# tjiiv-cprg/EPro-PnP

Hardware: AMD Instinct MI355X
Metric: PnP instances/sec (fwd+bwd, N=512 pts, 512 samples) (higher is better)
Workload: dtype f32; 1 GPU; C2 batched synthetic: 4096 objects/GPU x N=512 points, S=512 MC samples, K=4 AMIS iters, L=3 LM iters, EProPnP6DoF fwd+bwd; objects_per_gpu=4096, objects_total=4096, num_points=512, mc_samples=512, amis_iters=4, lm_iters=3, dof=6, parallelism=objects sharded x1, no data-path collective

## Files before the change

### epro-pnp_amd/csrc/amis_backward_mfma.hip

```cpp
#include "amis_common.h"
#include "dispatch.h"
#include "tuning.h"

namespace pnp {

template <int DOF, bool BOUNDS, int NPT, bool BF16>
constexpr int bwd_min_waves() { return (NPT <= 2) ? PNP_BWD_MINW : PNP_BWD_MINW4; }

template <int DOF, bool BOUNDS, int NPT, bool BF16 = false>
__global__ __launch_bounds__(512, (bwd_min_waves<DOF, BOUNDS, NPT, BF16>())) void amis_backward_mfma_kernel(Problem p, const float* __restrict__ pose_samples,
                                                                     const float* __restrict__ g_logw, int S,
                                                                     const float* __restrict__ pose_init,
                                                                     const float* __restrict__ g_init, int P16,
                                                                     float* __restrict__ gx3d, float* __restrict__ gx2d,
                                                                     float* __restrict__ gw2d, float* __restrict__ gdelta,
                                                                     int nsplit, float drop_eps, int gw_rows) {
  constexpr int PL = PoseLen<DOF>::value;
  typedef ProjOp<BF16> Proj;
  const int v = object_of_block(p.B * nsplit);
  if (v >= p.B * nsplit) return;
  const int b = v / nsplit, part = v - b * nsplit;
  const int T = (int)blockDim.x, tid = (int)threadIdx.x, lane = lane_id(), wv = wave_id(), W = T >> 6;

  PNP_PHASES_BEGIN(6);
  PNP_DYN_SMEM(float, smem);
  float* ptab = smem;
  float* wtab = ptab + 12 * P16;
  float* wraw = wtab + P16;
  int* idx = reinterpret_cast<int*>(wraw + P16);
  float* red = reinterpret_cast<float*>(idx + P16);
  float* hist = red + 80;
  float* gwl = hist + kDropHistFloats;
  const bool fold = (p.delta_stats != nullptr) && (nsplit == 1);
  const bool park = fold && (gw_rows >= p.N);

  float Kc[9], delta;
  Bounds bd;
  load_camera<BOUNDS>(p, b, Kc, bd, delta);
  const HuberScale hs = huber_scale(delta);
  const float zmin_v = to_vgpr(p.z_min), one_v = to_vgpr(1.0f);
  const float front_scale = to_vgpr(0x1p60f);
  const float front_off = to_vgpr(-nextafterf(p.z_min, -1.0f) * 0x1p60f);
  const float tiny_v = to_vgpr(1e-30f);

  const bool with_init = (pose_init != nullptr) && (g_init != nullptr);
  const int P = S + (with_init ? 1 : 0);
  const float g_init_b = with_init ? g_init[b] : 0.f;

  float amax = 0.f;
  for (int m = tid; m < P; m += T) {
    const float w = (m < S) ? -g_logw[(size_t)m * p.B + b] : g_init_b;
    wraw[m] = w;
    if (m < S) amax = fmaxf(amax, fabsf(w));
  }
  amax = block_max(amax, red);
  __syncthreads();
  PNP_PHASE(0);
  const float askip = mass_drop_threshold([&](int m) { return fabsf(wraw[m]); }, S, amax, drop_eps, hist);
  for (int m = tid; m < S; m += T)
    if (fabsf(wraw[m]) <= askip) wraw[m] = 0.f;
  __syncthreads();
  PNP_PHASE(1);
  if (wv == 0) {
    const int seg = (P + 63) >> 6;
    const int m0 = lane * seg, m1 = min(P, m0 + seg);
    int cnt = 0;
    for (int m = m0; m < m1; ++m) cnt += (wraw[m] != 0.f) ? 1 : 0;
    int* lcnt = reinterpret_cast<int*>(red);
    lcnt[lane] = cnt;
    wave_lds_fence();
    int off = 0, total = 0;
    for (int l = 0; l < 64; ++l) {
      const int c = lcnt[l];
      off += (l < lane) ? c : 0;
      total += c;
    }
    for (int m = m0; m < m1; ++m)
      if (wraw[m] != 0.f) idx[off++] = m;
    if (lane == 0) lcnt[64] = total;
  }
  __syncthreads();
  PNP_PHASE(2);
  const int nact = reinterpret_cast<const int*>(red)[64];
  const int ntile = (nact + 15) >> 4;
  for (int c = tid; c < ntile * 16; c += T) {
    float* dst = ptab + (c >> 2) * 48 + (c & 3);
    if (c < nact) {
      const int m = idx[c];
      const float* src = (m < S) ? pose_samples + ((size_t)m * p.B + b) * PL : pose_init + (size_t)b * PL;
      float ps[PL], R[9], KR[9], Kt[3];
#pragma unroll
      for (int i = 0; i < PL; ++i) ps[i] = src[i];
      pose_to_rot<DOF>(ps, R);
      compose_kr_kt(Kc, R, ps, KR, Kt);
#pragma unroll
      for (int r = 0; r < 3; ++r) {
        dst[(4 * r + 0) * 4] = KR[3 * r]; dst[(4 * r + 1) * 4] = KR[3 * r + 1]; dst[(4 * r + 2) * 4] = KR[3 * r + 2];
        dst[(4 * r + 3) * 4] = Kt[r];
      }
      wtab[c] = wraw[m];
    } else {
#pragma unroll
      for (int k = 0; k < 12; ++k) dst[k * 4] = (k == 11) ? 1.f : 0.f;
      wtab[c] = 0.f;
    }
  }
  __syncthreads();
  PNP_PHASE(3);

  const int col = lane & 15, kk = lane >> 4, g4 = kk * 4;
  float gd = 0.f;
  const int chunk_pts = W * NPT * 16;
  for (int c0 = part * chunk_pts; c0 < p.N; c0 += nsplit * chunk_pts) {
    typename Proj::T rB[NPT];
    float4 rW[NPT];
    f32x2 A1x[NPT], A1y[NPT], A2x[NPT], A2y[NPT];
    f32x2 gXv[NPT], gYv[NPT], gZv[NPT];
#pragma unroll
    for (int i = 0; i < NPT; ++i) {
      const Point q = load_point(p, b, c0 + (wv + W * i) * 16 + col);
      rB[i] = Proj::b((kk == 0) ? q.X : (kk == 1) ? q.Y : (kk == 2) ? q.Z : 1.0f);
      const float wu = q.wu * hs.inv_delta, wv = q.wv * hs.inv_delta;
      rW[i] = make_float4(wu, -q.u * wu, wv, -q.v * wv);
      A1x[i] = A1y[i] = A2x[i] = A2y[i] = f32x2{0.f, 0.f};
      gXv[i] = gYv[i] = gZv[i] = f32x2{0.f, 0.f};
    }
    f32x2 gsat2 = {0.f, 0.f};
    const floatx4 zero = {0.f, 0.f, 0.f, 0.f};
    const f32x2 tiny2 = {tiny_v, tiny_v};
    for (int t = 0; t < ntile; ++t) {
      const float* grp = ptab + (t * 4 + (col >> 2)) * 48 + (col & 3);
      const typename Proj::T ax = Proj::a(grp[kk * 4]), ay = Proj::a(grp[(4 + kk) * 4]), az = Proj::a(grp[(8 + kk) * 4]);
      const float4 aw4 = *reinterpret_cast<const float4*>(wtab + t * 16 + g4);
      const float4* rows = reinterpret_cast<const float4*>(ptab + (t * 4 + kk) * 48);
      const float4 kxx = rows[0], kxy = rows[1], kxz = rows[2], kyx = rows[4], kyy = rows[5], kyz = rows[6], kzx = rows[8], kzy = rows[9],
                   kzz = rows[10];
      constexpr bool kPipe = (NPT == 4);
      floatx4 hxn = zero, hyn = zero, hzn = zero;
      if (kPipe) {
        hxn = Proj::mma(ax, rB[0], zero); hyn = Proj::mma(ay, rB[0], zero); hzn = Proj::mma(az, rB[0], zero);
      }
#pragma unroll
      for (int i = 0; i < NPT; ++i) {
        floatx4 hx, hy, hz;
        if (kPipe) {
          hx = hxn; hy = hyn; hz = hzn;
          if (i + 1 < NPT) {
            hxn = Proj::mma(ax, rB[i + 1], zero);
            hyn = Proj::mma(ay, rB[i + 1], zero);
            hzn = Proj::mma(az, rB[i + 1], zero);
            sched_fence();
          }
        } else {
          hx = Proj::mma(ax, rB[i], zero);
          hy = Proj::mma(ay, rB[i], zero);
          hz = Proj::mma(az, rB[i], zero);
        }
        const float4 w4 = rW[i];
        const f32x2 wu2 = {w4.x, w4.x}, cu2 = {w4.y, w4.y}, wv2 = {w4.z, w4.z}, cv2 = {w4.w, w4.w};
#pragma unroll
        for (int h = 0; h < 2; ++h) {
          const f32x2 hx2 = {hx[2 * h], hx[2 * h + 1]}, hy2 = {hy[2 * h], hy[2 * h + 1]};
          const float hz0 = hz[2 * h], hz1 = hz[2 * h + 1];
          const f32x2 aw2 = h ? f32x2{aw4.z, aw4.w} : f32x2{aw4.x, aw4.y};
          const f32x2 rz2 = {fast_rcp(clamp_below(hz0, zmin_v)), fast_rcp(clamp_below(hz1, zmin_v))};
          f32x2 rx2, ry2, ghx2, ghy2, ghz2;
          f32x2 coef2, crx2, cry2;
          if (!BOUNDS) {
            const f32x2 wrx2 = rz2 * wu2, wry2 = rz2 * wv2;
            rx2 = fma2(hx2, wrx2, cu2);
            ry2 = fma2(hy2, wry2, cv2);
            const f32x2 s22 = fma2(rx2, rx2, fma2(ry2, ry2, tiny2));
            const f32x2 c12 = {sat_mul(fast_rsqrt(s22[0]), one_v), sat_mul(fast_rsqrt(s22[1]), one_v)};
            coef2 = aw2 * c12;
            gsat2 = fma2(aw2, f32x2{sat_mul(s22[0], one_v), sat_mul(s22[1], one_v)}, gsat2);
            crx2 = coef2 * rx2;
            cry2 = coef2 * ry2;
            ghx2 = crx2 * wrx2;
            ghy2 = cry2 * wry2;
            ghz2 = -rz2 * fma2(ghx2, hx2, ghy2 * hy2);
          } else {
            const f32x2 ppx2 = hx2 * rz2, ppy2 = hy2 * rz2;
            const f32x2 px2 = {clamp_lu(ppx2[0], bd.lbx, bd.ubx), clamp_lu(ppx2[1], bd.lbx, bd.ubx)};
            const f32x2 py2 = {clamp_lu(ppy2[0], bd.lby, bd.uby), clamp_lu(ppy2[1], bd.lby, bd.uby)};
            rx2 = fma2(px2, wu2, cu2);
            ry2 = fma2(py2, wv2, cv2);
            const f32x2 s22 = fma2(rx2, rx2, fma2(ry2, ry2, tiny2));
            const f32x2 c12 = {sat_mul(fast_rsqrt(s22[0]), one_v), sat_mul(fast_rsqrt(s22[1]), one_v)};
            coef2 = aw2 * c12;
            gsat2 = fma2(aw2, f32x2{sat_mul(s22[0], one_v), sat_mul(s22[1], one_v)}, gsat2);
            crx2 = coef2 * rx2;
            cry2 = coef2 * ry2;
            f32x2 gpx2 = crx2 * wu2, gpy2 = cry2 * wv2;
            gpx2 = f32x2{(px2[0] == ppx2[0]) ? gpx2[0] : 0.f, (px2[1] == ppx2[1]) ? gpx2[1] : 0.f};
            gpy2 = f32x2{(py2[0] == ppy2[0]) ? gpy2[0] : 0.f, (py2[1] == ppy2[1]) ? gpy2[1] : 0.f};
            ghx2 = gpx2 * rz2;
            ghy2 = gpy2 * rz2;
            ghz2 = fma2(-ghx2, ppx2, -(ghy2 * ppy2));
          }
          ghz2 = ghz2 * f32x2{sat_fma(hz0, front_scale, front_off), sat_fma(hz1, front_scale, front_off)};
          A2x[i] = fma2(crx2, rx2, A2x[i]);
          A2y[i] = fma2(cry2, ry2, A2y[i]);
          A1x[i] = fma2(coef2, rx2, A1x[i]);
          A1y[i] = fma2(coef2, ry2, A1y[i]);
          const f32x2 kxx2 = h ? f32x2{kxx.z, kxx.w} : f32x2{kxx.x, kxx.y}, kyx2 = h ? f32x2{kyx.z, kyx.w} : f32x2{kyx.x, kyx.y},
                      kzx2 = h ? f32x2{kzx.z, kzx.w} : f32x2{kzx.x, kzx.y};
          const f32x2 kxy2 = h ? f32x2{kxy.z, kxy.w} : f32x2{kxy.x, kxy.y}, kyy2 = h ? f32x2{kyy.z, kyy.w} : f32x2{kyy.x, kyy.y},
                      kzy2 = h ? f32x2{kzy.z, kzy.w} : f32x2{kzy.x, kzy.y};
          const f32x2 kxz2 = h ? f32x2{kxz.z, kxz.w} : f32x2{kxz.x, kxz.y}, kyz2 = h ? f32x2{kyz.z, kyz.w} : f32x2{kyz.x, kyz.y},
                      kzz2 = h ? f32x2{kzz.z, kzz.w} : f32x2{kzz.x, kzz.y};
          gXv[i] = fma2(kxx2, ghx2, fma2(kyx2, ghy2, fma2(kzx2, ghz2, gXv[i])));
          gYv[i] = fma2(kxy2, ghx2, fma2(kyy2, ghy2, fma2(kzy2, ghz2, gYv[i])));
          gZv[i] = fma2(kxz2, ghx2, fma2(kyz2, ghy2, fma2(kzz2, ghz2, gZv[i])));
        }
      }
    }
    const float gsat = gsat2[0] + gsat2[1];
    {
      float a2 = 0.f;
#pragma unroll
      for (int i = 0; i < NPT; ++i) a2 += (A2x[i][0] + A2x[i][1]) + (A2y[i][0] + A2y[i][1]);
      gd += a2 - gsat;
    }
    const int laneE = (int)f32_bits(to_vgpr(bits_f32((unsigned)lane)));
    const int colE = laneE & 15, g4E = (laneE >> 4) * 4;
    const float ind0 = (colE == 0) ? 1.f : 0.f, ind1 = (colE == 1) ? 1.f : 0.f, ind2 = (colE == 2) ? 1.f : 0.f,
                ind3 = (colE == 3) ? 1.f : 0.f;
#pragma unroll
    for (int i = 0; i < NPT; ++i) {
      floatx4 D1 = zero;
      D1 = mfma_16x16x4((gXv[i][0] + gXv[i][1]) * hs.delta_sq, ind0, D1);
      D1 = mfma_16x16x4((gYv[i][0] + gYv[i][1]) * hs.delta_sq, ind1, D1);
      D1 = mfma_16x16x4((gZv[i][0] + gZv[i][1]) * hs.delta_sq, ind2, D1);
      const float4 w4 = rW[i];
      floatx4 D2 = zero;
      const float a1x = A1x[i][0] + A1x[i][1], a1y = A1y[i][0] + A1y[i][1], a2x = A2x[i][0] + A2x[i][1], a2y = A2y[i][0] + A2y[i][1];
      D2 = mfma_16x16x4(-w4.x * a1x * hs.delta_sq, ind0, D2);
      D2 = mfma_16x16x4(-w4.z * a1y * hs.delta_sq, ind1, D2);
      D2 = mfma_16x16x4((w4.x != 0.f) ? a2x * hs.delta / w4.x : 0.f, ind2, D2);
      D2 = mfma_16x16x4((w4.z != 0.f) ? a2y * hs.delta / w4.z : 0.f, ind3, D2);
      const int nb = c0 + (wv + W * i) * 16 + g4E;
#pragma unroll
      for (int r = 0; r < 4; ++r) {
        const int n = nb + r;
        if (n < p.N) {
          const size_t o = (size_t)b * p.N + n;
          if (colE < 3) gx3d[o * 3 + colE] = D1[r];
          if (colE < 2) gx2d[o * 2 + colE] = D2[r];
          else if (colE < 4) {
            if (park) gwl[n * 2 + (colE - 2)] = D2[r]; else gw2d[o * 2 + (colE - 2)] = D2[r];
          }
        }
      }
    }
  }
  PNP_PHASE(4);
  float one[1] = {gd * hs.delta};
  block_sum<1>(one, red);
  if (tid == 0) gdelta[v] = one[0];
  if (fold) {
    const float add = (one[0] * p.delta_stats[(size_t)b * 4 + 1]) * (p.delta_relative / (2.0f * (float)p.N));
    __syncthreads();
    float* row = gw2d + (size_t)b * p.N * 2;
    if (park) {
      for (int i = tid; i < 2 * p.N; i += T) row[i] = gwl[i] + add;
    } else {
      for (int i = tid; i < 2 * p.N; i += T) row[i] += add;
    }
  }
  PNP_PHASE(5);
  PNP_PHASES_FLUSH(6);
}

int tuning_bwd_phase_cycles(unsigned long long* out, int reset) { return tuning::read_cycles(out, reset, false); }

template <class F>
static int dispatch_bwd_npt(int npt, F&& f) {
  switch (npt) {
    case 1: return f(ic<1>{});
    case 2: return f(ic<2>{});
    default: return f(ic<4>{});
  }
}

struct BwdPlan {
  int waves, npt, P16, gw_rows;
  size_t smem;
  bool bf16;
};

static int plan_amis_backward(const epropnp_problem* prob, int mc_samples, bool with_init, int nsplit, BwdPlan* out) {
  const int B = prob->num_obj, N = prob->num_pts;
  const int P = mc_samples + (with_init ? 1 : 0);
  const int P16 = ((P + 15) / 16) * 16 + 16;
  size_t smem = sizeof(float) * (15 * (size_t)P16 + 80 + kDropHistFloats);
  if (smem > 160 * 1024) return 1;
  int gw_rows = 0;
  if (prob->delta_stats != nullptr && nsplit == 1 && 3 * (smem + sizeof(float) * 2 * (size_t)N) <= 160 * 1024) {
    gw_rows = N;
    smem += sizeof(float) * 2 * (size_t)N;
  }
  const int ptiles = (N + 15) / 16;
  int waves = (B < 512 && ptiles > 16) ? 8 : 4, npt = 1;
  while (npt < 4 && waves * npt < ptiles) npt *= 2;
  if (has_bounds(prob) && waves == 4 && npt == 4 && B >= 2 * device_cu_count() && 3 * smem <= 160 * 1024) npt = 2;
  if (nsplit > 1) {
    waves = 4; npt = 1;
    while (npt < 4 && waves * npt * nsplit < ptiles) npt *= 2;
  }
  { int ov[2]; if (tune_ints("bwd_mfma", ov, 2) && ov[0] >= 1 && ov[0] <= 8 && (ov[1] == 1 || ov[1] == 2 || ov[1] == 4)) { waves = ov[0]; npt = ov[1]; } }
  bool bf16 = true;
  if (const char* e = getenv("EPROPNP_BWD_PROJ")) bf16 = (e[0] == 'f') ? false : (e[0] == 'b' ? true : bf16);
  out->waves = waves; out->npt = npt; out->P16 = P16; out->gw_rows = gw_rows; out->smem = smem; out->bf16 = bf16;
  return 0;
}

int plan_amis_backward_record(const epropnp_problem* prob, int mc_samples, int with_init, int nsplit, int32_t* out) {
  BwdPlan plan;
  const bool valu = (backward_valu_forced() && nsplit == 1) || plan_amis_backward(prob, mc_samples, with_init != 0, nsplit, &plan) != 0;
  out[0] = valu ? 0 : plan.waves; out[1] = valu ? 0 : plan.npt; out[2] = valu ? 0 : plan.bf16; out[3] = valu ? 0 : plan.gw_rows > 0;
  out[4] = valu;
  return EPROPNP_OK;
}

int launch_amis_backward_mfma(const epropnp_problem* prob, const float* pose_samples, const float* grad_logweights,
                              int mc_samples, const float* pose_init, const float* grad_cost_init, float* grad_x3d,
                              float* grad_x2d, float* grad_w2d, float* grad_delta, int nsplit, hipStream_t st) {
  const Problem d = to_device_problem(prob);
  BwdPlan plan;
  if (plan_amis_backward(prob, mc_samples, pose_init && grad_cost_init, nsplit, &plan)) return 1;
  const int waves = plan.waves, npt = plan.npt, P16 = plan.P16, gw_rows = plan.gw_rows;
  const size_t smem = plan.smem;
  const bool bf16 = plan.bf16;
  const dim3 grid(padded_object_grid(d.B * nsplit)), block(64 * waves);
  dispatch_dof_bounds(prob->dof, has_bounds(prob), [&](auto DOF, auto BND) -> int {
    auto launch = [&](auto kern) -> int {
      allow_dynamic_lds((const void*)kern, smem);
      PNP_LAUNCH(kern, grid, block, smem, st, d, pose_samples, grad_logweights, mc_samples, pose_init, grad_cost_init, P16,
                 grad_x3d, grad_x2d, grad_w2d, grad_delta, nsplit, backward_drop_eps(), gw_rows);
      return 0;
    };
    if (bf16)
      return (npt == 1)   ? launch(amis_backward_mfma_kernel<decltype(DOF)::value, decltype(BND)::value, 1, true>)
             : (npt == 2) ? launch(amis_backward_mfma_kernel<decltype(DOF)::value, decltype(BND)::value, 2, true>)
                          : launch(amis_backward_mfma_kernel<decltype(DOF)::value, decltype(BND)::value, 4, true>);
    return dispatch_bwd_npt(npt, [&](auto NPT) -> int {
      return launch(amis_backward_mfma_kernel<decltype(DOF)::value, decltype(BND)::value, decltype(NPT)::value>);
    });
  });
  return check_launch("amis_backward_mfma_kernel");
}

}
```

Measured before the change: 2.947 million instances/s.

## Restructure backward prologue: parallel compaction, log-bin mass threshold, prefetched poses and points

After: 2.964 million instances/s, median of 6. About the same (+0.6%).

```diff
diff --git a/epro-pnp_amd/csrc/amis_backward_mfma.hip b/epro-pnp_amd/csrc/amis_backward_mfma.hip
--- a/epro-pnp_amd/csrc/amis_backward_mfma.hip
+++ b/epro-pnp_amd/csrc/amis_backward_mfma.hip
@@ -22,13 +22,12 @@
   const int b = v / nsplit, part = v - b * nsplit;
   const int T = (int)blockDim.x, tid = (int)threadIdx.x, lane = lane_id(), wv = wave_id(), W = T >> 6;
 
-  PNP_PHASES_BEGIN(6);
+  PNP_PHASES_BEGIN(8);
   PNP_DYN_SMEM(float, smem);
   float* ptab = smem;
   float* wtab = ptab + 12 * P16;
   float* wraw = wtab + P16;
-  int* idx = reinterpret_cast<int*>(wraw + P16);
-  float* red = reinterpret_cast<float*>(idx + P16);
+  float* red = wraw + 2 * P16;
   float* hist = red + 80;
   float* gwl = hist + kDropHistFloats;
   const bool fold = (p.delta_stats != nullptr) && (nsplit == 1);
@@ -47,70 +46,142 @@
   const int P = S + (with_init ? 1 : 0);
   const float g_init_b = with_init ? g_init[b] : 0.f;
 
+  const int col = lane & 15, kk = lane >> 4, g4 = kk * 4;
+  const int chunk_pts = W * NPT * 16;
+  const int seg = (P + T - 1) / T, m0 = tid * seg, m1 = min(P, m0 + seg);
+  constexpr int kPre = 3;
+  auto weight_of = [&](int m) { return (m < S) ? -g_logw[(size_t)m * p.B + b] : g_init_b; };
+  auto pose_of = [&](int m) { return (m < S) ? pose_samples + ((size_t)m * p.B + b) * PL : pose_init + (size_t)b * PL; };
   float amax = 0.f;
-  for (int m = tid; m < P; m += T) {
-    const float w = (m < S) ? -g_logw[(size_t)m * p.B + b] : g_init_b;
+  for (int m = m0; m < m1; ++m) {
+    const float w = weight_of(m);
     wraw[m] = w;
     if (m < S) amax = fmaxf(amax, fabsf(w));
   }
-  amax = block_max(amax, red);
+  float psr[kPre][PL];
+#pragma unroll
+  for (int r = 0; r < kPre; ++r) {
+    const float* src = pose_of(min(m0 + r, P - 1));
+#pragma unroll
+    for (int i = 0; i < PL; ++i) psr[r][i] = (m0 + r < m1) ? src[i] : 0.f;
+  }
+  Point qn[NPT];
+#pragma unroll
+  for (int i = 0; i < NPT; ++i) qn[i] = load_point(p, b, part * chunk_pts + (wv + W * i) * 16 + col);
+
+  unsigned long long* bins = reinterpret_cast<unsigned long long*>(ptab);
+  unsigned char* cnts = reinterpret_cast<unsigned char*>(red + 8);
+  int* gsum = reinterpret_cast<int*>(red + 8 + 128);
+  amax = wave_max(amax);
+  if (lane == 0) red[wv] = amax;
+  if (tid < 64) bins[tid] = 0ull;
   __syncthreads();
+  amax = red[0];
+  for (int k = 1; k < W; ++k) amax = fmaxf(amax, red[k]);
   PNP_PHASE(0);
-  const float askip = mass_drop_threshold([&](int m) { return fabsf(wraw[m]); }, S, amax, drop_eps, hist);
-  for (int m = tid; m < S; m += T)
-    if (fabsf(wraw[m]) <= askip) wraw[m] = 0.f;
+  const bool usable = (amax > 0.f) && (amax < INFINITY);
+  const float inv = usable ? 1.0f / amax : 0.f;
+  for (int m = m0; m < min(m1, S); ++m) {
+    const float rel = fminf(fabsf(wraw[m]) * inv, 1.0f);
+    int k = (rel > 0.f) ? (int)(-__builtin_amdgcn_logf(rel)) : 63;
+    k = min(max(k, 0), 63);
+    const unsigned long long q = (unsigned long long)(rel * 0x1p40f);
+    if (q != 0ull) atomicAdd(&bins[k], q);
+  }
   __syncthreads();
+  float askip;
+  {
+    unsigned long long c = 0ull;
+#pragma unroll
+    for (int j = 0; j < 8; ++j) {
+      const int k = (lane & ~7) + j;
+      const unsigned long long v = bins[k];
+      c += (k >= lane) ? v : 0ull;
+    }
+    const int clo = (int)(unsigned)c, chi = (int)(unsigned)(c >> 32);
+#pragma unroll
+    for (int g = 1; g < 8; ++g) {
+      const unsigned long long gt = ((unsigned long long)(unsigned)wave_bcast(chi, 8 * g) << 32) | (unsigned)wave_bcast(clo, 8 * g);
+      c += ((lane >> 3) < g) ? gt : 0ull;
+    }
+    const unsigned long long total =
+        ((unsigned long long)(unsigned)wave_bcast((int)(unsigned)(c >> 32), 0) << 32) | (unsigned)wave_bcast((int)(unsigned)c, 0);
+    const unsigned long long budget = (unsigned long long)((double)total * (double)drop_eps);
+    const unsigned kmin = wave_min_u32((c <= budget) ? (unsigned)lane : 64u);
+    askip = (usable && kmin < 64u) ? ldexpf(amax, -(int)kmin) : 0.f;
+  }
   PNP_PHASE(1);
-  if (wv == 0) {
-    const int seg = (P + 63) >> 6;
-    const int m0 = lane * seg, m1 = min(P, m0 + seg);
+  auto kept = [&](int m, float w) { return (m < S) ? !(fabsf(w) <= askip) : (w != 0.f); };
+  {
     int cnt = 0;
-    for (int m = m0; m < m1; ++m) cnt += (wraw[m] != 0.f) ? 1 : 0;
-    int* lcnt = reinterpret_cast<int*>(red);
-    lcnt[lane] = cnt;
-    wave_lds_fence();
-    int off = 0, total = 0;
-    for (int l = 0; l < 64; ++l) {
-      const int c = lcnt[l];
-      off += (l < lane) ? c : 0;
-      total += c;
-    }
-    for (int m = m0; m < m1; ++m)
-      if (wraw[m] != 0.f) idx[off++] = m;
-    if (lane == 0) lcnt[64] = total;
+    for (int m = m0; m < m1; ++m) cnt += kept(m, wraw[m]) ? 1 : 0;
+    cnts[tid] = (unsigned char)cnt;
   }
   __syncthreads();
+  auto byte_sum = [](unsigned x) { const unsigned y = (x & 0x00ff00ffu) + ((x >> 8) & 0x00ff00ffu); return (int)((y & 0xffffu) + (y >> 16)); };
+  if (tid < (T >> 4)) {
+    const float4 cw = *reinterpret_cast<const float4*>(cnts + 16 * tid);
+    gsum[tid] = (byte_sum(f32_bits(cw.x)) + byte_sum(f32_bits(cw.y))) + (byte_sum(f32_bits(cw.z)) + byte_sum(f32_bits(cw.w)));
+  }
+  __syncthreads();
+  int off = 0, nsum = 0;
+  for (int g = 0; g < (T >> 4); ++g) {
+    const int c = gsum[g];
+    off += (g < (tid >> 4)) ? c : 0;
+    nsum += c;
+  }
+  const int nact = __builtin_amdgcn_readfirstlane(nsum);
+  {
+    const float4 cw = *reinterpret_cast<const float4*>(cnts + (tid & ~15));
+    const unsigned w4[4] = {f32_bits(cw.x), f32_bits(cw.y), f32_bits(cw.z), f32_bits(cw.w)};
+#pragma unroll
+    for (int i = 0; i < 4; ++i) {
+      const int nb = min(max((tid & 15) - 4 * i, 0), 4);
+      off += byte_sum(w4[i] & ((nb >= 4) ? 0xffffffffu : ((1u << (8 * nb)) - 1u)));
+    }
+  }
   PNP_PHASE(2);
-  const int nact = reinterpret_cast<const int*>(red)[64];
   const int ntile = (nact + 15) >> 4;
-  for (int c = tid; c < ntile * 16; c += T) {
+  auto place = [&](int c, const float (&ps)[PL], float w) {
     float* dst = ptab + (c >> 2) * 48 + (c & 3);
-    if (c < nact) {
-      const int m = idx[c];
-      const float* src = (m < S) ? pose_samples + ((size_t)m * p.B + b) * PL : pose_init + (size_t)b * PL;
-      float ps[PL], R[9], KR[9], Kt[3];
+    float R[9], KR[9], Kt[3];
+    pose_to_rot<DOF>(ps, R);
+    compose_kr_kt(Kc, R, ps, KR, Kt);
+#pragma unroll
+    for (int r = 0; r < 3; ++r) {
+      dst[(4 * r + 0) * 4] = KR[3 * r]; dst[(4 * r + 1) * 4] = KR[3 * r + 1]; dst[(4 * r + 2) * 4] = KR[3 * r + 2];
+      dst[(4 * r + 3) * 4] = Kt[r];
+    }
+    wtab[c] = w;
+  };
+#pragma unroll
+  for (int r = 0; r < kPre; ++r) {
+    const int m = m0 + r;
+    if (m < m1) {
+      const float w = wraw[m];
+      if (kept(m, w)) place(off++, psr[r], w);
+    }
+  }
+  for (int m = m0 + kPre; m < m1; ++m) {
+    const float w = wraw[m];
+    if (kept(m, w)) {
+      const float* src = pose_of(m);
+      float ps[PL];
 #pragma unroll
       for (int i = 0; i < PL; ++i) ps[i] = src[i];
-      pose_to_rot<DOF>(ps, R);
-      compose_kr_kt(Kc, R, ps, KR, Kt);
-#pragma unroll
-      for (int r = 0; r < 3; ++r) {
-        dst[(4 * r + 0) * 4] = KR[3 * r]; dst[(4 * r + 1) * 4] = KR[3 * r + 1]; dst[(4 * r + 2) * 4] = KR[3 * r + 2];
-        dst[(4 * r + 3) * 4] = Kt[r];
-      }
-      wtab[c] = wraw[m];
-    } else {
-#pragma unroll
-      for (int k = 0; k < 12; ++k) dst[k * 4] = (k == 11) ? 1.f : 0.f;
-      wtab[c] = 0.f;
-    }
+      place(off++, ps, w);
+    }
+  }
+  for (int c = nact + tid; c < ntile * 16; c += T) {
+    float* dst = ptab + (c >> 2) * 48 + (c & 3);
+#pragma unroll
+    for (int k = 0; k < 12; ++k) dst[k * 4] = (k == 11) ? 1.f : 0.f;
+    wtab[c] = 0.f;
   }
   __syncthreads();
   PNP_PHASE(3);
 
-  const int col = lane & 15, kk = lane >> 4, g4 = kk * 4;
   float gd = 0.f;
-  const int chunk_pts = W * NPT * 16;
   for (int c0 = part * chunk_pts; c0 < p.N; c0 += nsplit * chunk_pts) {
     typename Proj::T rB[NPT];
     float4 rW[NPT];
@@ -118,13 +189,14 @@
     f32x2 gXv[NPT], gYv[NPT], gZv[NPT];
 #pragma unroll
     for (int i = 0; i < NPT; ++i) {
-      const Point q = load_point(p, b, c0 + (wv + W * i) * 16 + col);
+      const Point q = qn[i];
       rB[i] = Proj::b((kk == 0) ? q.X : (kk == 1) ? q.Y : (kk == 2) ? q.Z : 1.0f);
       const float wu = q.wu * hs.inv_delta, wv = q.wv * hs.inv_delta;
       rW[i] = make_float4(wu, -q.u * wu, wv, -q.v * wv);
       A1x[i] = A1y[i] = A2x[i] = A2y[i] = f32x2{0.f, 0.f};
       gXv[i] = gYv[i] = gZv[i] = f32x2{0.f, 0.f};
     }
+    PNP_PHASE(7);
     f32x2 gsat2 = {0.f, 0.f};
     const floatx4 zero = {0.f, 0.f, 0.f, 0.f};
     const f32x2 tiny2 = {tiny_v, tiny_v};
@@ -215,6 +287,9 @@
         }
       }
     }
+    PNP_PHASE(4);
+#pragma unroll
+    for (int i = 0; i < NPT; ++i) qn[i] = load_point(p, b, c0 + nsplit * chunk_pts + (wv + W * i) * 16 + col);
     const float gsat = gsat2[0] + gsat2[1];
     {
       float a2 = 0.f;
@@ -253,8 +328,8 @@
         }
       }
     }
-  }
-  PNP_PHASE(4);
+    PNP_PHASE(6);
+  }
   float one[1] = {gd * hs.delta};
   block_sum<1>(one, red);
   if (tid == 0) gdelta[v] = one[0];
@@ -269,7 +344,7 @@
     }
   }
   PNP_PHASE(5);
-  PNP_PHASES_FLUSH(6);
+  PNP_PHASES_FLUSH(8);
 }
 
 int tuning_bwd_phase_cycles(unsigned long long* out, int reset) { return tuning::read_cycles(out, reset, false); }
```
